# xarray-contrib/xeofs

Hardware: AMD Instinct MI355X
Metric: EOF randomized-SVD GB/s (algorithmic: 16 passes x n x p x 4 B per fit / fit time) (higher is better)
Workload: dtype f32 data, split-fp16 MFMA (f16x3+f16x3), f32 accumulate

## Files before the change

include/eofx.h:

```cpp
#ifndef EOFX_H
#define EOFX_H

#include <stdint.h>

#ifdef __cplusplus
extern "C" {
#endif

#define EOFX_ABI_VERSION 1
#define EOFX_MAX_SKETCH 256

#define EOFX_OK 0
#define EOFX_ERR_ARG (-1)
#define EOFX_ERR_HIP (-2)
#define EOFX_ERR_PARTIAL_NAN (-3)
#define EOFX_ERR_NAN_MISMATCH (-4)
#define EOFX_ERR_RANK (-5)
#define EOFX_ERR_LINALG (-6)
#define EOFX_ERR_NOMEM (-7)
#define EOFX_ERR_SHAPE (-8)

typedef struct eofx_ctx eofx_ctx;
typedef struct eofx_mat eofx_mat;

// ... 84 lines not shown
int eofx_ctx_last_iterations(const eofx_ctx *ctx, int *iterations);

int eofx_project_f32(eofx_ctx *ctx, const eofx_mat *m, const float *V, int k, float *out);
int eofx_reconstruct_f32(eofx_ctx *ctx, const float *S, const float *V, int64_t n, int64_t p,
                         int k, float *out);

int eofx_crosscov_rsvd_f32(eofx_ctx *ctx, const eofx_mat *x, const eofx_mat *y, int k,
                           int n_oversamples, int n_iter, const float *omega, int flip, float *Q1,
                           float *s, float *Q2, float *scores1, float *scores2, float *norm1,
                           float *norm2, double *tsc);
typedef const float *(*eofx_sketch_fn)(void *user);
int eofx_crosscov_rsvd_lazy_f32(eofx_ctx *ctx, const eofx_mat *x, const eofx_mat *y, int k, int n_oversamples,
                                int n_iter, eofx_sketch_fn omega_fn, void *omega_user, int flip, float *Q1, float *s,
                                float *Q2, float *scores1, float *scores2, float *norm1, float *norm2, double *tsc);

int eofx_panel_tmul_f32(eofx_ctx *ctx, const eofx_mat *m, const float *Zn, float *Yp, int L,
                        int precision);
int eofx_panel_mul_f32(eofx_ctx *ctx, const eofx_mat *m, const float *Yp, float *Wn, int L,
                       int precision);
int eofx_panel_gram_f64(eofx_ctx *ctx, const float *P, int64_t rows_pad, int L, double *G);
int eofx_panel_cholqr_f32(eofx_ctx *ctx, const float *P, int64_t rows_pad, int L, int l,
                          const double *G, float *out);
int eofx_panel_rinv_f64(eofx_ctx *ctx, const double *G, int L, int l, double *Rinv);
int eofx_panel_matmul_f32(eofx_ctx *ctx, const float *P, int64_t rows_pad, int L,
                          const double *M, int Lo, float *out);
int eofx_panel_colminmax_f32(eofx_ctx *ctx, const float *P, int64_t rows, int L, float *mx,
                             float *mn);
int eofx_panel_export_f32(eofx_ctx *ctx, const float *P, int64_t rows, int L, int k,
                          const double *sign, float *dst);
int eofx_panel_import_f32(eofx_ctx *ctx, const float *src, int64_t rows, int l, float *P,
                          int64_t rows_pad, int L);

int eofx_hilbert_f32(eofx_ctx *ctx, const eofx_mat *a, int padding, double decay_factor,
                     eofx_mat **out_imag, eofx_mat **out_real);
int eofx_mat_sumsq_f64(eofx_ctx *ctx, const eofx_mat *m, double *out);
int eofx_panel_rownorm_f64(eofx_ctx *ctx, const float *P, int64_t rows, int L, double *out);
int eofx_mat_feature_norms_f64(eofx_ctx *ctx, const eofx_mat *m, double *out);
int eofx_mat_sample_norms_f64(eofx_ctx *ctx, const eofx_mat *m, double *out);
int eofx_resample_f32(eofx_ctx *ctx, const eofx_mat *src, const int64_t *rows, int64_t n_rows, int center,
                      eofx_mat **out, double *mean, double *total_variance);
int eofx_panel_bootstrap_f32(eofx_ctx *ctx, const float *P_in, int64_t n, int64_t rows_pad, int L, const int64_t *idx,
                             const int64_t *order, const int64_t *rowptr, int transpose, float *P_out);
int eofx_lag_stats_f64(eofx_ctx *ctx, const eofx_mat *m, int tau, int embedding, double *mean, double *total_variance);
int eofx_lag_tmul_f32(eofx_ctx *ctx, const eofx_mat *m, int tau, int embedding, const double *mean, const float *Zn, int L,
                      float *Ye, int prec);
int eofx_lag_mul_f32(eofx_ctx *ctx, const eofx_mat *m, int tau, int embedding, const double *mean, const float *Ye, int L,
// ... 58 lines not shown
```

xeofs_amd/_lib.py:

```python

from __future__ import annotations

import ctypes as C
import os

import numpy as np

_HERE = os.path.dirname(os.path.abspath(__file__))
LIB_PATH = os.environ.get("EOFX_LIB") or os.path.join(_HERE, "lib", "libeofx.so")

EOFX_OK = 0
ERR_ARG, ERR_HIP, ERR_PARTIAL_NAN, ERR_NAN_MISMATCH, ERR_RANK, ERR_LINALG, ERR_NOMEM, ERR_SHAPE = (
    -1, -2, -3, -4, -5, -6, -7, -8)

_vp = C.c_void_p
_i64 = C.c_int64
_int = C.c_int
_pi64 = C.POINTER(C.c_int64)
_pd = C.POINTER(C.c_double)

SKETCH_FN = C.CFUNCTYPE(C.c_void_p, C.c_void_p)

ALLREDUCE_FN = C.CFUNCTYPE(C.c_int, C.c_void_p, C.c_void_p, C.c_int64, C.c_int, C.c_int, C.c_void_p)

# ... 8 lines not shown
    "eofx_ctx_set_precision": (_int, [_vp, _int, _int]),
    "eofx_ctx_profile": (_int, [_vp, _int]),
    "eofx_ctx_profile_read": (_int, [_vp, _pi64, _pd, _pd, _pd]),
    "eofx_ctx_profile_by_kernel": (_int, [_vp, _pi64, _pd]),
    "eofx_preprocess_f32": (_int, [_vp, _vp, _i64, _i64, _int, _int, _vp, _int, C.POINTER(_vp),
                                   _vp, _vp, _vp, _vp, _pi64, _pi64, _pd]),
    "eofx_apply_f32": (_int, [_vp, _vp, _i64, _i64, _vp, _vp, _vp, _vp, _int, C.POINTER(_vp), _vp, _pi64]),
    "eofx_mat_from_dense_f32": (_int, [_vp, _vp, _i64, _i64, _i64, C.POINTER(_vp)]),
    "eofx_mat_destroy": (_int, [_vp, _vp]),
    "eofx_mat_shape": (_int, [_vp, _pi64, _pi64, _pi64, _pi64]),
    "eofx_mat_download_f32": (_int, [_vp, _vp, _vp]),
    "eofx_rsvd_f32": (_int, [_vp, _vp, _int, _int, _int, _vp, _int, _vp, _vp, _vp]),
    "eofx_project_f32": (_int, [_vp, _vp, _vp, _int, _vp]),
    "eofx_reconstruct_f32": (_int, [_vp, _vp, _vp, _i64, _i64, _int, _vp]),
    "eofx_crosscov_rsvd_f32": (_int, [_vp, _vp, _vp, _int, _int, _int, _vp, _int, _vp, _vp, _vp, _vp,
                                      _vp, _vp, _vp, _pd]),
    "eofx_crosscov_rsvd_lazy_f32": (_int, [_vp, _vp, _vp, _int, _int, _int, SKETCH_FN, _vp, _int, _vp, _vp, _vp, _vp,
                                           _vp, _vp, _vp, _pd]),
    "eofx_panel_tmul_f32": (_int, [_vp, _vp, _vp, _vp, _int, _int]),
    "eofx_panel_mul_f32": (_int, [_vp, _vp, _vp, _vp, _int, _int]),
    "eofx_panel_gram_f64": (_int, [_vp, _vp, _i64, _int, _vp]),
    "eofx_panel_cholqr_f32": (_int, [_vp, _vp, _i64, _int, _int, _vp, _vp]),
    "eofx_panel_rinv_f64": (_int, [_vp, _vp, _int, _int, _vp]),
    "eofx_panel_matmul_f32": (_int, [_vp, _vp, _i64, _int, _vp, _int, _vp]),
    "eofx_panel_colminmax_f32": (_int, [_vp, _vp, _i64, _int, _vp, _vp]),
    "eofx_panel_export_f32": (_int, [_vp, _vp, _i64, _int, _int, _vp, _vp]),
    "eofx_panel_import_f32": (_int, [_vp, _vp, _i64, _int, _vp, _i64, _int]),
    "eofx_hilbert_f32": (_int, [_vp, _vp, _int, C.c_double, C.POINTER(_vp), C.POINTER(_vp)]),
    "eofx_mat_sumsq_f64": (_int, [_vp, _vp, _pd]),
    "eofx_fit_f32": (_int, [_vp, _vp, _i64, _i64, _int, _int, _vp, _int, _int, _int, _int, _vp, _i64, _int,
                            C.POINTER(_vp), _vp, _vp, _vp, _vp, _pi64, _pi64, _pd, _vp, _vp, _vp, C.POINTER(C.c_int)]),
    "eofx_fit_first_f32": (_int, [_vp, _vp, _i64, _i64, _int, _int, _vp, _int, _vp, _int, _int, _vp, C.POINTER(_vp),
                                  _vp, _vp, _vp, _vp, _pi64, _pi64, _pd, C.POINTER(C.c_int)]),
    "eofx_ctx_fit_info": (_int, [_vp, _pd]),
    "eofx_ctx_last_iterations": (_int, [_vp, C.POINTER(_int)]),
    "eofx_comm_unique_id": (_int, [C.c_char_p]),
    "eofx_ctx_comm_init_rccl": (_int, [_vp, C.c_char_p, _int, _int]),
    "eofx_ctx_comm_set_callback": (_int, [_vp, ALLREDUCE_FN, _vp, _int, _int]),
    "eofx_ctx_comm_clear": (_int, [_vp]),
    "eofx_ctx_comm_stats": (_int, [_vp, _pi64, _pi64, _pd]),
    "eofx_ctx_comm_selftest": (_int, [_vp, C.POINTER(C.c_int)]),
    "eofx_ctx_comm_probe": (_int, [_vp, _int, _vp, _vp, _int, _vp, _vp]),
    "eofx_fit_sharded_f32": (_int, [_vp, _vp, _i64, _i64, _i64, _int, _int, _vp, _int, _int, _int, _vp, _i64, _int,
                                    C.POINTER(_vp), _vp, _vp, _vp, _pd, _vp, _vp, _vp]),
    "eofx_ctx_comm_allreduce_f64": (_int, [_vp, _vp, _i64, _int]),
    "eofx_crosscov_rsvd_sharded_f32": (_int, [_vp, _vp, _vp, _i64, _i64, _i64, _i64, _int, _int, _int, _vp, _int, _vp, _vp,
# ... 103 lines not shown
```

xeofs_amd/csrc/eofx_abi.hip:

```cpp
#include <chrono>
#include "eofx_hfft.hpp"
#include "eofx_kernels.hpp"
#include "eofx_fit.hpp"
#include "eofx_gram.hpp"
#include "eofx_axb_dma.hpp"
#include "eofx_hosteig.hpp"
#include "eofx_lag.hpp"
#include "eofx_gw.hpp"
#include "eofx_spca.hpp"
#include "eofx_lagcov.hpp"
#ifndef EOFX_AXB_DMA_DEFAULT
#define EOFX_AXB_DMA_DEFAULT 1
#endif

#if !defined(__HIP_DEVICE_COMPILE__)
#include <immintrin.h>
#endif
#include <algorithm>
#include <array>
#include <atomic>
#include <cmath>
#include <complex>
#include <cstdarg>
#include <cstdio>
// ... 74 lines not shown
    int kind;
    ProfEvent(hipEvent_t a, hipEvent_t b, int k = 0) : first(a), second(b), kind(k) {}
  };
  std::vector<ProfEvent> prof_events;
  int64_t prof_kind_launches[3] = {0, 0, 0};
  double prof_kind_ms[3] = {0.0, 0.0, 0.0};
  double prof_flops = 0.0;
  double prof_bytes = 0.0;
  unsigned* amax_slots = nullptr;
  int amax_next = 0, amax_depth = 0;
  std::vector<std::pair<const float*, const unsigned*>> amax_known;
  double* pinned = nullptr;
  struct GramPlanDev {
    int nti = 0, ntj = 0, nst = 0;
    bool sym = false;
    GramPlan pl;
    GramItem* items = nullptr;
    int2* tiles = nullptr;
  };
  std::vector<GramPlanDev*> gram_plans;
  _Float16* axb_planes = nullptr;
  size_t axb_planes_bytes = 0;
  int axb_dma = -1;
  double fit_info[4] = {0.0, 0.0, 0.0, 0.0};
  int last_iters = 0;
  EofxComm* comm = nullptr;
};
constexpr int EOFX_AMAX_SLOTS = 1024;
constexpr int EOFX_HILBERT_OP_MAX_N = 16384;
constexpr size_t EOFX_PINNED_DOUBLES = 2 * 256 * 256 + 64;

struct eofx_mat {
  int64_t n = 0, p = 0, n_pad = 0, p_pad = 0;
  float* X = nullptr;
  float* Xt = nullptr;
  const float* raw = nullptr;
  float* raw_owned = nullptr;
  size_t raw_owned_bytes = 0;
  int64_t raw_ld = 0;
  float* aff = nullptr;
  unsigned* absmax_dev = nullptr;
  float absmax = 0.f;
  bool masked = false;
  int64_t p_valid = 0;
  int* act = nullptr;
  int64_t n_act = -1;
// ... 141 lines not shown
    std::lock_guard<std::mutex> g(g_fence[device].reg_mu);
    g_fence[device].ctxs.push_back(ctx);
  }
  *out = ctx;
  return EOFX_OK;
}
extern "C" int eofx_ctx_destroy(eofx_ctx* ctx) {
  if (!ctx) return EOFX_OK;
  {
    FenceGuard fence(ctx, false);
    if (ctx->device >= 0 && ctx->device < EOFX_MAX_DEVICES) {
      std::lock_guard<std::mutex> g(g_fence[ctx->device].reg_mu);
      auto& v = g_fence[ctx->device].ctxs;
      v.erase(std::remove(v.begin(), v.end(), ctx), v.end());
    }
  }
  (void)hipSetDevice(ctx->device);
  if (ctx->arena) {
    (void)hipStreamSynchronize(ctx->stream);
    (void)hipFree(ctx->arena);
  }
  pool_trim(ctx);
  if (ctx->amax_slots) (void)hipFree(ctx->amax_slots);
  if (ctx->pinned) (void)hipHostFree(ctx->pinned);
  for (auto& e : ctx->fft_plans) {
    hipfftDestroy((hipfftHandle)e.second.first);
    hipfftDestroy((hipfftHandle)e.second.second);
  }
  (void)eofx_ctx_comm_clear(ctx);
  if (ctx->axb_planes) (void)hipFree(ctx->axb_planes);
  for (auto* g : ctx->gram_plans) {
    if (g->items) (void)hipFree(g->items);
    if (g->tiles) (void)hipFree(g->tiles);
    delete g;
  }
  for (auto& h : ctx->hops) (void)eofx_mat_destroy(ctx, h.m);
  ctx->hops.clear();
  for (auto& h : ctx->hsetups) {
    if (h.chat) (void)hipFree(h.chat);
    if (h.hperm) (void)hipFree(h.hperm);
    if (h.u) (void)hipFree(h.u);
  }
  delete ctx;
  return EOFX_OK;
}
extern "C" int eofx_ctx_set_stream(eofx_ctx* ctx, void* stream) {
// ... 582 lines not shown
    if (masked)
      hipLaunchKernelGGL((axb_f16_kernel<4, 0, true>), dim3(gx, nfull), dim3(256), 0, ctx->stream, raw, ld, (int)rows, cols, aff, aff_ld, Y,
                         L, out, L, rows_pad, K, plan.kps, plan.S, rt, 0, a_scale, bmax, act);
    else
      hipLaunchKernelGGL(axb_f16_kernel<4>, dim3(gx, nfull), dim3(256), 0, ctx->stream, raw, ld, (int)rows, cols, aff, aff_ld, Y, L, out,
                         L, rows_pad, K, plan.kps, plan.S, rt, 0, a_scale, bmax);
    KCHK();
  }
  if (!dma && rem) {
    if (masked)
      hipLaunchKernelGGL((axb_f16_kernel<2, 0, true>), dim3(gx, 1), dim3(256), 0, ctx->stream, raw, ld, (int)rows, cols, aff, aff_ld, Y, L,
                         out, L, rows_pad, K, plan.kps, plan.S, rt, nfull * 64, a_scale, bmax, act);
    else
      hipLaunchKernelGGL(axb_f16_kernel<2>, dim3(gx, 1), dim3(256), 0, ctx->stream, raw, ld, (int)rows, cols, aff, aff_ld, Y, L, out,
                         L, rows_pad, K, plan.kps, plan.S, rt, nfull * 64, a_scale, bmax);
    KCHK();
  }
  if (ctx->profile) {
    HIPCHK(hipEventRecord(ev1, ctx->stream));
    ctx->prof_events.emplace_back(ev0, ev1, 1);
    ctx->prof_flops += 2.0 * (double)K * (double)rows_pad * (double)L;
    ctx->prof_bytes += (double)K * (double)rows * 4.0 * (nfull + (rem ? 1 : 0));
  }
  if (plan.S > 1) {
    const int64_t count4 = rows_pad * L / 4;
    hipLaunchKernelGGL(splitk_reduce_kernel, dim3((int)std::min<int64_t>((count4 + 255) / 256, amax_out ? 2048 : 4096)), dim3(256), 0,
                       ctx->stream, out, W, count4, plan.S, amax_out);
    KCHK();
  }
  return EOFX_OK;
}

static int gram_parts(int64_t rows, int L) {
  const int64_t by_rows = std::min<int64_t>((rows + 127) / 128, 256);
  const int64_t by_mem = ((int64_t)128 << 20) / ((int64_t)L * L * 8);
  if (const char* ev = std::getenv("EOFX_GRAM_PARTS")) return std::max(1, atoi(ev));
  return (int)std::max<int64_t>(1, std::min(by_rows, std::max<int64_t>(by_mem, 1)));
}

static int launch_gram(eofx_ctx* ctx, const float* P, int64_t rows, int L, double* G) {
  const int nb = (L + 63) / 64;
  const int nbx = gram_parts(rows, L);
  ArenaScope scope(ctx);
  ARENA(double, part, (size_t)nbx * L * L);
  hipLaunchKernelGGL(gram_mfma_kernel, dim3(nbx, nb * nb), dim3(256), 0, ctx->stream, P, rows, L, part);
  KCHK();
  const int64_t count = (int64_t)L * L;
// ... 73 lines not shown
    if (dead[c]) continue;
    X[(size_t)c * l + c] = 1.0 / A[(size_t)c * l + c];
    for (int r = c - 1; r >= 0; --r) {
      double sum = 0.0;
      for (int t = r + 1; t <= c; ++t) sum += A[(size_t)r * l + t] * X[(size_t)t * l + c];
      X[(size_t)r * l + c] = -sum / A[(size_t)r * l + r];
    }
  }
  for (int r = 0; r < L; ++r)
    for (int c = 0; c < L; ++c) Rinv[(size_t)r * L + c] = (r < l && c < l) ? X[(size_t)r * l + c] : 0.0;
}

static int launch_rinv(eofx_ctx* ctx, const double* G, int L, int l, double* Rinv);
static size_t rinv_blocked_bytes(int l);
static bool matmul_nt_ok(int64_t rows, int L, int Lo);
static size_t matmul_nt_scratch(eofx_ctx* ctx, int64_t rows, int L, int Lo);
static int launch_matmul_nt(eofx_ctx* ctx, const float* P, int64_t rows, int L, const double* Mx, int Lo, float* out);
static int launch_cholqr(eofx_ctx* ctx, const float* P, int64_t rows, int L, int l, const double* G,
                         float* out) {
  ArenaScope scope(ctx);
  ARENA(double, Rinv, (size_t)L * L);
  CHK(launch_rinv(ctx, G, L, l, Rinv));
  return launch_matmul(ctx, P, rows, L, Rinv, L, out, true);
}

static int launch_colminmax(eofx_ctx* ctx, const float* P, int64_t rows, int L, float* mx, float* mn) {
  const int nparts = (int)std::max<int64_t>(1, std::min<int64_t>((rows + 127) / 128, 1024));
  ArenaScope scope(ctx);
  ARENA(float, pmx, (size_t)nparts * L);
  ARENA(float, pmn, (size_t)nparts * L);
  hipLaunchKernelGGL(colminmax_part_kernel, dim3(nparts, (L + 63) / 64), dim3(256), 0, ctx->stream, P,
                     rows, L, pmx, pmn);
  KCHK();
  hipLaunchKernelGGL(colminmax_final_kernel, dim3((L + 63) / 64), dim3(256), 0, ctx->stream, pmx, pmn,
                     nparts, L, mx, mn);
  KCHK();
  return EOFX_OK;
}

static int export_panel(eofx_ctx* ctx, const float* P, int64_t rows, int L, int k, const double* sign,
                        float* dst) {
  if (!dst) return EOFX_OK;
  ArenaScope scope(ctx);
  double* dsign = nullptr;
  if (sign) {
    dsign = arena_alloc<double>(ctx, k);
// ... 808 lines not shown
  ENTER(ctx);
  CHK(arena_reserve(ctx, atb_scratch_bytes(m->n_pad, round_up(m->p, ATB_KG), L)));
  return panel_mul(ctx, m, Yp, Wn, L, prec);
}
extern "C" int eofx_panel_gram_f64(eofx_ctx* ctx, const float* P, int64_t rows_pad, int L, double* G) {
  if (!ctx || !P || !G || L % 32) return set_err(ctx, EOFX_ERR_ARG, "bad argument");
  ENTER(ctx);
  CHK(arena_reserve(ctx, (size_t)(4 * gram_parts(rows_pad, L) + 1) * L * L * sizeof(double)));
  return launch_gram(ctx, P, rows_pad, L, G);
}
extern "C" int eofx_panel_cholqr_f32(eofx_ctx* ctx, const float* P, int64_t rows_pad, int L, int l,
                                     const double* G, float* out) {
  if (!ctx || !P || !G || !out || P == out) return set_err(ctx, EOFX_ERR_ARG, "bad argument");
  ENTER(ctx);
  CHK(arena_reserve(ctx, (size_t)2 * L * L * sizeof(double) + (l > 64 ? rinv_blocked_bytes(l) : 0)));
  return launch_cholqr(ctx, P, rows_pad, L, l, G, out);
}
extern "C" int eofx_panel_rinv_f64(eofx_ctx* ctx, const double* G, int L, int l, double* Rinv) {
  if (!ctx || !G || !Rinv || L <= 0 || l <= 0 || l > L || G == Rinv) return set_err(ctx, EOFX_ERR_ARG, "bad argument");
  ENTER(ctx);
  if (l > 64) CHK(arena_reserve(ctx, rinv_blocked_bytes(l)));
  return launch_rinv(ctx, G, L, l, Rinv);
}
extern "C" int eofx_panel_matmul_f32(eofx_ctx* ctx, const float* P, int64_t rows_pad, int L,
                                     const double* M, int Lo, float* out) {
  if (!ctx || !P || !M || !out || P == out) return set_err(ctx, EOFX_ERR_ARG, "bad argument");
  ENTER(ctx);
  if (matmul_nt_ok(rows_pad, L, Lo)) {
    const size_t need = matmul_nt_scratch(ctx, rows_pad, L, Lo);
    if (need && arena_reserve(ctx, need) == EOFX_OK) return launch_matmul_nt(ctx, P, rows_pad, L, M, Lo, out);
  }
  return launch_matmul(ctx, P, rows_pad, L, M, Lo, out);
}
extern "C" int eofx_panel_colminmax_f32(eofx_ctx* ctx, const float* P, int64_t rows, int L, float* mx,
                                        float* mn) {
  if (!ctx || !P || !mx || !mn) return set_err(ctx, EOFX_ERR_ARG, "bad argument");
  if (L <= 0 || L % 4 || rows < 0)
    return set_err(ctx, EOFX_ERR_ARG, "colminmax: L=%d must be a positive multiple of 4, rows=%lld non-negative", L, (long long)rows);
  ENTER(ctx);
  CHK(arena_reserve(ctx, (size_t)2 * 1024 * L * sizeof(float) + 4096));
  return launch_colminmax(ctx, P, rows, L, mx, mn);
}
extern "C" int eofx_panel_export_f32(eofx_ctx* ctx, const float* P, int64_t rows, int L, int k,
                                     const double* sign, float* dst) {
  if (!ctx || !P || !dst || k > L) return set_err(ctx, EOFX_ERR_ARG, "bad argument");
  ENTER(ctx);
  CHK(arena_reserve(ctx, (size_t)rows * k * sizeof(float) + 8192));
  return export_panel(ctx, P, rows, L, k, sign, dst);
}
extern "C" int eofx_panel_import_f32(eofx_ctx* ctx, const float* src, int64_t rows, int l, float* P,
                                     int64_t rows_pad, int L) {
  if (!ctx || !P || !src || l > L || rows > rows_pad) return set_err(ctx, EOFX_ERR_ARG, "bad argument");
  if (L <= 0 || L % 4 || l < 0 || rows < 0)
    return set_err(ctx, EOFX_ERR_ARG, "import: L=%d must be a positive multiple of 4, l=%d and rows=%lld non-negative", L, l, (long long)rows);
  ENTER(ctx);
  CHK(arena_reserve(ctx, (size_t)rows * l * sizeof(float) + 8192));
  return import_panel(ctx, src, rows, l, P, rows_pad, L);
}

struct LinOp {
  int64_t tall, small, tall_pad, small_pad;
  std::function<int(const float*, float*, int, int)> fwd;
  std::function<int(const float*, float*, int, int)> bwd;
  std::function<int(double*, int64_t)> reduce_tall_gram;
  std::function<int(double*, int64_t)> reduce_small_gram;
  int64_t rule_tall_pad = 0;
};

struct RsvdOut {
  float* Tvec;
  float* Svec;
  int Lo;
  std::vector<double> s;
  int64_t tall_pad = 0, small_pad = 0;
};

static int rsvd_auto_iters(int k, int64_t n, int64_t p) {
  return ((double)k < 0.1 * (double)std::min(n, p)) ? 7 : 4;
}

constexpr size_t EOFX_ORTH_TALL_BYTES = (size_t)16 << 20;
constexpr double EOFX_PEAKED_RATIO = 30.0;
static bool orth_tall_rule(int64_t tall_pad, int L, int prec_power) {
  if (std::getenv("EOFX_FORCE_ORTH_TALL")) return true;
  return prec_power == EOFX_PREC_F64 || (size_t)tall_pad * L * sizeof(float) <= EOFX_ORTH_TALL_BYTES;
}
extern "C" int eofx_orth_tall_rule(int64_t tall_rows_pad, int L, int prec_power) {
  return orth_tall_rule(tall_rows_pad, L, prec_power) ? 1 : 0;
}
// ... 125 lines not shown
  bool first_done = false;
  auto fwd = [&](const float* z, float* y, int prec) -> int {
    if (first_fwd && !first_done) {
      first_done = true;
      return (*first_fwd)(z, y, L);
    }
    first_done = true;
    return op.fwd(z, y, L, prec);
  };
  auto gram_tall = [&](const float* Pn, double* Gout) -> int {
    CHK(launch_gram(ctx, Pn, op.tall_pad, L, Gout));
    return op.reduce_tall_gram ? op.reduce_tall_gram(Gout, (int64_t)L * L) : EOFX_OK;
  };
  auto gram_small = [&](const float* Pn, double* Gout) -> int {
    CHK(launch_gram(ctx, Pn, op.small_pad, L, Gout));
    return op.reduce_small_gram ? op.reduce_small_gram(Gout, (int64_t)L * L) : EOFX_OK;
  };
  const int pp = ctx->prec_power, pf = ctx->prec_final;
  const bool orth_always = orth_tall_rule(op.rule_tall_pad > 0 ? op.rule_tall_pad : op.tall_pad, L, pp);
  bool orth_rest = orth_always;
  hipEvent_t peaked_ev = nullptr;
  bool peaked_pending = false;
  int rc = EOFX_OK;
  for (int it = 0; it < (range ? 0 : n_iter) && rc == EOFX_OK; ++it) {
    rc = fwd(Zs, Yt, pp);
    if (rc != EOFX_OK) break;
    if (peaked_pending) {
      peaked_pending = false;
      if (hipEventSynchronize(peaked_ev) != hipSuccess) rc = set_err(ctx, EOFX_ERR_HIP, "event wait failed");
      else orth_rest = eofx_peaked_spectrum(pin, L, l) != 0;
      if (rc != EOFX_OK) break;
    }
    if (it == 0 || orth_rest) {
      if ((rc = gram_tall(Yt, G)) != EOFX_OK) break;
      if ((rc = launch_cholqr(ctx, Yt, op.tall_pad, L, l, G, Qt)) != EOFX_OK) break;
      rc = op.bwd(Qt, Ws, L, pp);
    } else {
      rc = op.bwd(Yt, Ws, L, pp);
    }
    if (rc != EOFX_OK) break;
    const bool ask = it == 0 && !orth_always && n_iter > 1;
    if ((rc = gram_small(Ws, ask ? G0 : G)) != EOFX_OK) break;
    if (ask) {
      if (hipMemcpyAsync(pin, G0, sizeof(double) * L * L, hipMemcpyDeviceToHost, ctx->stream) != hipSuccess ||
          (!peaked_ev && hipEventCreateWithFlags(&peaked_ev, hipEventDisableTiming) != hipSuccess) ||
          hipEventRecord(peaked_ev, ctx->stream) != hipSuccess) {
        rc = set_err(ctx, EOFX_ERR_HIP, "asynchronous Gram download failed");
        break;
      }
      peaked_pending = true;
    }
    rc = launch_cholqr(ctx, Ws, op.small_pad, L, l, ask ? G0 : G, Zs);
  }
  if (peaked_ev) {
    if (peaked_pending) (void)hipEventSynchronize(peaked_ev);
    (void)hipEventDestroy(peaked_ev);
  }
  if (rc != EOFX_OK) return rc;
  if (range) CHK((*range)(Zs, Yt, L));
  else CHK(fwd(Zs, Yt, pp));
  CHK(gram_tall(Yt, G));
  CHK(launch_cholqr(ctx, Yt, op.tall_pad, L, l, G, Qt));
  CHK(gram_tall(Qt, G));
  CHK(launch_rinv(ctx, G, L, l, R2));
  CHK(op.bwd(Qt, Zs, L, pf));
  CHK(launch_matmul(ctx, Zs, op.small_pad, L, R2, L, Ws));
  CHK(gram_small(Ws, G));
  double* hG = pin;
  double* hR2 = pin + (size_t)L * L;
  HIPCHK(hipMemcpyAsync(hG, G, sizeof(double) * L * L, hipMemcpyDeviceToHost, ctx->stream));
  HIPCHK(hipMemcpyAsync(hR2, R2, sizeof(double) * L * L, hipMemcpyDeviceToHost, ctx->stream));
  HIPCHK(hipStreamSynchronize(ctx->stream));
  std::vector<double> Gl((size_t)l * l), w(l), Uh((size_t)l * l);
  for (int i = 0; i < l; ++i)
    for (int j = 0; j < l; ++j) {
// ... 212 lines not shown
                             const float* omega, int flip, float* U, float* s, float* V) {
  if (!ctx || !m || !omega || k <= 0 || n_oversamples < 0) return set_err(ctx, EOFX_ERR_ARG, "bad argument");
  ENTER(ctx);
  const int64_t n = m->n, p = m->p, r = std::min(n, p);
  if (k > r)
    return set_err(ctx, EOFX_ERR_RANK,
                   "n_modes must be less than or equal to the rank of the dataset (rank = %lld).", (long long)r);
  const int l_req = k + n_oversamples;
  const int l = (int)std::min<int64_t>(l_req, r);
  if (l > EOFX_MAX_SKETCH)
    return set_err(ctx, EOFX_ERR_ARG, "sketch width k+n_oversamples = %d > %d is not supported", l, EOFX_MAX_SKETCH);
  if (n_iter < 0) n_iter = rsvd_auto_iters(k, n, p);
  const bool transposed = n < p;
  LinOp op;
  if (transposed) {
    op = {p, n, m->p_pad, m->n_pad,
          [&](const float* z, float* y, int L, int pr) { return panel_tmul(ctx, m, z, y, L, pr); },
          [&](const float* y, float* w, int L, int pr) { return panel_mul(ctx, m, y, w, L, pr); }};
  } else {
    op = {n, p, m->n_pad, m->p_pad,
          [&](const float* z, float* y, int L, int pr) { return panel_mul(ctx, m, z, y, L, pr); },
          [&](const float* y, float* w, int L, int pr) { return panel_tmul(ctx, m, y, w, L, pr); }};
  }
  CHK(arena_reserve(ctx, rsvd_scratch_bytes(op.tall_pad, op.small_pad, l, k)));
  ArenaScope scope(ctx);
  std::vector<float> om_clamped;
  const float* om = omega;
  if (l == r) {
    om_clamped.assign((size_t)op.small * l, 0.f);
    for (int64_t i = 0; i < l; ++i) om_clamped[(size_t)i * l + i] = 1.f;
    om = om_clamped.data();
  } else if (l != l_req) {
    if (is_device_ptr(omega)) return set_err(ctx, EOFX_ERR_ARG, "omega must be a host pointer");
    om_clamped.resize((size_t)op.small * l);
    for (int64_t i = 0; i < op.small; ++i)
      for (int j = 0; j < l; ++j) om_clamped[(size_t)i * l + j] = omega[(size_t)i * l_req + j];
    om = om_clamped.data();
  }
  RsvdOut ro;
  CHK(rsvd_core(ctx, op, k, l, n_iter, om, ro));
  return rsvd_finish(ctx, ro, transposed, n, p, k, flip, U, s, V);
}

struct FitFirst {
  eofx_ctx* ctx = nullptr;
  const float* Xd = nullptr;
// ... 208 lines not shown
  }
};

static bool fit_first_eligible(const eofx_ctx* ctx, const float* Xdev, int64_t n, int64_t P, int l) {
  return ctx->keep_raw == 2 && ctx->prec_power == EOFX_PREC_F16X3 && n < P && l > 0 && l < n && round_up(l, 32) <= 64 &&
         l % 32 != 0 && P % 4 == 0 && ((uintptr_t)Xdev % 16) == 0 && n < ((int64_t)1 << 31) && !std::getenv("EOFX_NO_FUSED_FIT");
}

static int fit_fused(eofx_ctx* ctx, const float* Xd, int64_t n, int64_t P, int center, int standardize,
                     const double* feat_weights, int k, int l, int n_iter, const float* omega, int flip,
                     eofx_mat** out, double* mean, double* std_, double* total_variance, float* U, float* s, float* V,
                     uint8_t* valid_feature, int64_t* p_valid) {
  const int64_t p_pad = round_up(P, ATB_BM), n_pad = round_up(n, ATB_BM);
  CHK(arena_reserve(ctx, rsvd_scratch_bytes(p_pad, n_pad, l, k) + FitFirst::bytes(n, P, l)));
  ArenaScope scope(ctx);
  FitFirst ff;
  int rc = ff.prepare(ctx, Xd, n, P, center, standardize, feat_weights, l);
  if (rc != EOFX_OK) return rc;
  FirstFwd first = [&](const float* Zs, float* Yt, int LL) -> int { return ff.run(Zs, Yt, LL); };
  const eofx_mat* m = ff.m;
  LinOp op = {P, n, p_pad, n_pad,
              [&](const float* z, float* y, int LL, int pr) { return panel_tmul(ctx, m, z, y, LL, pr); },
              [&](const float* y, float* w, int LL, int pr) { return panel_mul(ctx, m, y, w, LL, pr); }};
  RsvdOut ro;
  rc = rsvd_core(ctx, op, k, l, n_iter, omega, ro, &first);
  if (rc != EOFX_OK) return rc;
  CHK(rsvd_finish(ctx, ro, true, n, P, k, flip, U, s, V));
  CHK(ff.valid_features(valid_feature));
  if (p_valid) *p_valid = ff.m->masked ? ff.m->p_valid : P;
  return ff.finish(mean, std_, total_variance, out);
}

extern "C" int eofx_fit_first_f32(eofx_ctx* ctx, const float* X, int64_t n, int64_t P, int center, int standardize,
                                  const double* feat_weights, int check_nans, const float* Zn, int L, int l, float* Yp,
                                  eofx_mat** out, double* mean, double* std_, uint8_t* valid_feature, uint8_t* valid_sample,
                                  int64_t* n_out, int64_t* p_out, double* total_variance, int* fused) {
  if (!ctx || !X || !out || !Zn || !Yp || n <= 0 || P <= 0 || L <= 0 || L % 32 || l <= 0 || l > L)
    return set_err(ctx, EOFX_ERR_ARG, "bad argument");
  ENTER(ctx);
  if (fused) *fused = 0;
  ctx->fit_info[0] = ctx->fit_info[1] = ctx->fit_info[2] = 0.0;
  Staged st;
  CHK(stage_input(ctx, X, (size_t)n * P, st));
  if (fit_first_eligible(ctx, st.dev, n, P, l) && round_up(l, 32) == L) {
    CHK(arena_reserve(ctx, FitFirst::bytes(n, P, l) + atb_scratch_bytes(round_up(P, ATB_BM), round_up(n, ATB_KG), L)));
    ArenaScope scope(ctx);
// ... 3519 lines not shown
```

xeofs_amd/csrc/eofx_kernels.hpp:

```cpp
#pragma once
#include <hip/hip_runtime.h>
#include <stdint.h>

namespace eofx {

typedef float f32x16 __attribute__((ext_vector_type(16)));
typedef float f32x4 __attribute__((ext_vector_type(4)));
typedef float f32x2 __attribute__((ext_vector_type(2)));

__device__ __forceinline__ void aff_split(double sh, float& hi, float& lo) {
  hi = (float)sh;
  lo = (float)(sh - (double)hi);
}
__device__ __forceinline__ float aff_map(float x, float sh_hi, float sh_lo, float scale) {
  return ((x - sh_hi) - sh_lo) * scale;
}
__device__ __forceinline__ float aff_fma(float x, float sh_hi, float s, float nls) {
  return __builtin_fmaf(x - sh_hi, s, nls);
}

__device__ __forceinline__ void amax_commit(float mx, unsigned* __restrict__ amax_out) {
  __shared__ float amax_red_[16];
#pragma unroll
  for (int o = 32; o > 0; o >>= 1) mx = fmaxf(mx, __shfl_xor(mx, o));
// ... 1174 lines not shown

__global__ __launch_bounds__(256) void cproj_embed_kernel(const double* __restrict__ C, int nb, int LP, double* __restrict__ E) {
  const int h = LP / 2;
  const int64_t total = (int64_t)nb * h * h;
  for (int64_t t = (int64_t)blockIdx.x * blockDim.x + threadIdx.x; t < total; t += (int64_t)gridDim.x * blockDim.x) {
    const int b = (int)(t / (h * h)), i = (int)(t / h % h), j = (int)(t % h);
    const double* Cb = C + (int64_t)b * LP * LP;
    double* Eb = E + (int64_t)b * LP * LP;
    const double rr = Cb[i * LP + j], ii = Cb[(h + i) * LP + h + j], ri = Cb[i * LP + h + j], ir = Cb[(h + i) * LP + j];
    const double cr = rr + ii, ci = ri - ir;
    Eb[i * LP + j] = cr;
    Eb[(h + i) * LP + j] = -ci;
    Eb[i * LP + h + j] = ci;
    Eb[(h + i) * LP + h + j] = cr;
  }
}

__device__ __forceinline__ double rl_f64(double v, int lane) {
  const int lo = __builtin_amdgcn_readlane(__double2loint(v), lane);
  const int hi = __builtin_amdgcn_readlane(__double2hiint(v), lane);
  return __hiloint2double(hi, lo);
}

__global__ __launch_bounds__(256) void chol_rinv_kernel(const double* __restrict__ G, int L, int l,
                                                         double* __restrict__ Rinv, double tol,
                                                         const double* __restrict__ d0_ext = nullptr,
                                                         unsigned long long* __restrict__ prof = nullptr) {
#define EOFX_RINV_T(i) do { if (prof && threadIdx.x == 0) prof[i] = wall_clock64(); } while (0)
  EOFX_RINV_T(0);
  __shared__ double A[64][65];
  __shared__ double X[64][65];
  __shared__ double d0s[64], pivs[64];
  __shared__ double Tm[3][16][17];
  __shared__ int dead[64];
  const int tid = threadIdx.x;
  for (int i = tid; i < 64 * 64; i += 256) {
    const int r = i >> 6, c = i & 63;
    double v = (r == c) ? 1.0 : 0.0;
    if (r <= c && c < l) v = G[(int64_t)r * L + c];
    A[r][c] = v;
  }
  if (tid < 64) {
    d0s[tid] = (tid < l) ? (d0_ext ? d0_ext[tid] : G[(int64_t)tid * L + tid]) : 1.0;
    pivs[tid] = 1.0;
    dead[tid] = 0;
  }
  __syncthreads();
  EOFX_RINV_T(1);
  for (int jb = 0; jb < l; jb += 8) {
    const int je = jb + 8;
// ... 71 lines not shown
#pragma unroll 16
          for (int m = 0; m < 16; ++m) t += A[16 * i + rr][16 * k + m] * X[16 * k + m][16 * j + cc];
        Tm[i][rr][cc] = t;
      }
      __syncthreads();
      for (int i = 0; i + d < 4; ++i) {
        const int j = i + d;
        double x = 0.0;
#pragma unroll 16
        for (int m = 0; m < 16; ++m) x += X[16 * i + rr][16 * i + m] * Tm[i][m][cc];
        X[16 * i + rr][16 * j + cc] = -x;
      }
      __syncthreads();
    }
  }
  __syncthreads();
  EOFX_RINV_T(3);
  for (int i = tid; i < 64 * 64; i += 256) {
    const int r = i >> 6, c = i & 63;
    if (r < L && c < L) Rinv[(int64_t)r * L + c] = (r <= c && c < l && !dead[c]) ? X[r][c] : 0.0;
  }
  EOFX_RINV_T(4);
#undef EOFX_RINV_T
}

template <bool TA>
__global__ __launch_bounds__(256) void dgemm64_kernel(const double* __restrict__ A, int lda, const double* B, int ldb,
                                                       double* C, int ldc, int K, double alpha, double beta, int upper,
                                                       int64_t sA = 0, int64_t sB = 0, int64_t sC = 0) {
  __shared__ double As[16][65], Bs[16][65];
  const int bx = blockIdx.x, by = blockIdx.y;
  if (upper && by > bx) return;
  A += (int64_t)blockIdx.z * sA;
  B += (int64_t)blockIdx.z * sB;
  C += (int64_t)blockIdx.z * sC;
  const int tx = threadIdx.x & 15, ty = threadIdx.x >> 4;
  double acc[4][4];
#pragma unroll
  for (int i = 0; i < 4; ++i)
#pragma unroll
    for (int j = 0; j < 4; ++j) acc[i][j] = 0.0;
  for (int k0 = 0; k0 < K; k0 += 16) {
#pragma unroll
    for (int e = 0; e < 4; ++e) {
      const int idx = threadIdx.x + 256 * e;
      if (TA) {
// ... 1340 lines not shown
```

xeofs_amd/engine.py:

```python

from __future__ import annotations

import contextlib
import ctypes as C
import numbers

import numpy as np

from . import _lib
from ._lib import ptr, raise_for


def _f32c(a):
    if isinstance(a, np.ndarray):
        return np.ascontiguousarray(a, dtype=np.float32)
    if hasattr(a, "data_ptr"):
        import torch

        if a.dtype != torch.float32 or not a.is_contiguous():
            a = a.to(torch.float32).contiguous()
        return a
    return np.ascontiguousarray(np.asarray(a), dtype=np.float32)


# ... 725 lines not shown
    L = Yp.shape[1]
    if out is None:
        out = torch.empty((mat.n_pad, L), dtype=torch.float32, device=Yp.device)
    raise_for(ctx.lib.eofx_panel_mul_f32(ctx.handle, mat.handle, ptr(Yp), ptr(out), L, _lib.PREC[prec]), ctx.handle)
    return out


def panel_gram(ctx: Context, P, out=None):
    torch = _torch()
    L = P.shape[1]
    if out is None:
        out = torch.empty((L, L), dtype=torch.float64, device=P.device)
    raise_for(ctx.lib.eofx_panel_gram_f64(ctx.handle, ptr(P), P.shape[0], L, ptr(out)), ctx.handle)
    return out


def panel_cholqr(ctx: Context, P, l: int, G, out=None):
    torch = _torch()
    if out is None:
        out = torch.empty_like(P)
    raise_for(ctx.lib.eofx_panel_cholqr_f32(ctx.handle, ptr(P), P.shape[0], P.shape[1], int(l), ptr(G), ptr(out)),
              ctx.handle)
    return out


def panel_rinv(ctx: Context, G, l: int):
    torch = _torch()
    out = torch.empty_like(G)
    raise_for(ctx.lib.eofx_panel_rinv_f64(ctx.handle, ptr(G), G.shape[0], int(l), ptr(out)), ctx.handle)
    return out


def panel_matmul(ctx: Context, P, M, out=None):
    torch = _torch()
    Lo = M.shape[1]
    if out is None:
        out = torch.empty((P.shape[0], Lo), dtype=torch.float32, device=P.device)
    raise_for(ctx.lib.eofx_panel_matmul_f32(ctx.handle, ptr(P), P.shape[0], P.shape[1], ptr(M), Lo, ptr(out)),
              ctx.handle)
    return out


def panel_colminmax(ctx: Context, P, rows: int):
    torch = _torch()
    L = P.shape[1]
    mx = torch.empty(L, dtype=torch.float32, device=P.device)
# ... 341 lines not shown
```

Baseline: 5905.

## Fuse split-K reduce, small Gram, and Cholesky inverse into one kernel

In the randomized-SVD power iteration, the backward product's split-K reduction is deferred and fused with the small-side Gram computation (f64 MFMA), a last-block ticket reduction of per-block Gram partials, and the Cholesky/R-inverse into a single kernel launch. The old path ran a separate reduce kernel, a Gram kernel, and a cholqr path. This removes several kernel launches and one full read of the reduced panel. In exchange it adds a global atomic ticket with release/acquire fences and last-block serial work, and exposes a test entry point plus an environment switch to turn it off.

```diff
diff --git a/include/eofx.h b/include/eofx.h
--- a/include/eofx.h
+++ b/include/eofx.h
@@ -130,6 +130,8 @@
 int eofx_panel_cholqr_f32(eofx_ctx *ctx, const float *P, int64_t rows_pad, int L, int l,
                           const double *G, float *out);
 int eofx_panel_rinv_f64(eofx_ctx *ctx, const double *G, int L, int l, double *Rinv);
+int eofx_panel_small_step_f32(eofx_ctx *ctx, const float *part, int splits, int64_t rows_pad, int l, int fused,
+                              float *Ws, double *G, double *Rinv, float *Zs, unsigned *amax);
 int eofx_panel_matmul_f32(eofx_ctx *ctx, const float *P, int64_t rows_pad, int L,
                           const double *M, int Lo, float *out);
 int eofx_panel_colminmax_f32(eofx_ctx *ctx, const float *P, int64_t rows, int L, float *mx,
diff --git a/xeofs_amd/_lib.py b/xeofs_amd/_lib.py
--- a/xeofs_amd/_lib.py
+++ b/xeofs_amd/_lib.py
@@ -54,6 +54,7 @@
     "eofx_panel_gram_f64": (_int, [_vp, _vp, _i64, _int, _vp]),
     "eofx_panel_cholqr_f32": (_int, [_vp, _vp, _i64, _int, _int, _vp, _vp]),
     "eofx_panel_rinv_f64": (_int, [_vp, _vp, _int, _int, _vp]),
+    "eofx_panel_small_step_f32": (_int, [_vp, _vp, _int, _i64, _int, _int, _vp, _vp, _vp, _vp, _vp]),
     "eofx_panel_matmul_f32": (_int, [_vp, _vp, _i64, _int, _vp, _int, _vp]),
     "eofx_panel_colminmax_f32": (_int, [_vp, _vp, _i64, _int, _vp, _vp]),
     "eofx_panel_export_f32": (_int, [_vp, _vp, _i64, _int, _int, _vp, _vp]),
diff --git a/xeofs_amd/csrc/eofx_abi.hip b/xeofs_amd/csrc/eofx_abi.hip
--- a/xeofs_amd/csrc/eofx_abi.hip
+++ b/xeofs_amd/csrc/eofx_abi.hip
@@ -120,6 +120,13 @@
   _Float16* axb_planes = nullptr;
   size_t axb_planes_bytes = 0;
   int axb_dma = -1;
+  struct AxbDefer {
+    const float* W = nullptr;
+    const float* part = nullptr;
+    int S = 0;
+  };
+  AxbDefer* axb_defer = nullptr;
+  unsigned* step_ticket = nullptr;
   double fit_info[4] = {0.0, 0.0, 0.0, 0.0};
   int last_iters = 0;
   EofxComm* comm = nullptr;
@@ -307,6 +314,7 @@
   }
   pool_trim(ctx);
   if (ctx->amax_slots) (void)hipFree(ctx->amax_slots);
+  if (ctx->step_ticket) (void)hipFree(ctx->step_ticket);
   if (ctx->pinned) (void)hipHostFree(ctx->pinned);
   for (auto& e : ctx->fft_plans) {
     hipfftDestroy((hipfftHandle)e.second.first);
@@ -935,7 +943,10 @@
     ctx->prof_flops += 2.0 * (double)K * (double)rows_pad * (double)L;
     ctx->prof_bytes += (double)K * (double)rows * 4.0 * (nfull + (rem ? 1 : 0));
   }
-  if (plan.S > 1) {
+  if (plan.S > 1 && ctx->axb_defer && ctx->axb_defer->W == W) {
+    ctx->axb_defer->part = out;
+    ctx->axb_defer->S = plan.S;
+  } else if (plan.S > 1) {
     const int64_t count4 = rows_pad * L / 4;
     hipLaunchKernelGGL(splitk_reduce_kernel, dim3((int)std::min<int64_t>((count4 + 255) / 256, amax_out ? 2048 : 4096)), dim3(256), 0,
                        ctx->stream, out, W, count4, plan.S, amax_out);
@@ -1055,6 +1066,24 @@
   ARENA(double, Rinv, (size_t)L * L);
   CHK(launch_rinv(ctx, G, L, l, Rinv));
   return launch_matmul(ctx, P, rows, L, Rinv, L, out, true);
+}
+
+static int launch_small_step(eofx_ctx* ctx, const float* part, int splits, float* Ws, int64_t rows, int l, double* gpart, double* G,
+                             double* Rinv, unsigned* amax_ws) {
+  if (rows <= 0 || rows >= ((int64_t)1 << 40) || l <= 0 || l > 64 || splits < 1) return set_err(ctx, EOFX_ERR_ARG, "small step: bad geometry");
+  if (!ctx->step_ticket) {
+    HIPCHK(hipMalloc((void**)&ctx->step_ticket, 256));
+    HIPCHK(hipMemsetAsync(ctx->step_ticket, 0, 256, ctx->stream));
+  }
+  const int nbx = gram_parts(rows, 64);
+  hipLaunchKernelGGL(small_step_kernel, dim3(nbx), dim3(256), 0, ctx->stream, part, splits, Ws, part != Ws ? 1 : 0, rows, l, gpart, G, Rinv,
+                     1e-13, ctx->step_ticket, amax_ws);
+  KCHK();
+  return EOFX_OK;
+}
+static bool small_step_off() {
+  const char* ev = std::getenv("EOFX_SMALL_STEP");
+  return ev && atoi(ev) == 0;
 }
 
 static int launch_colminmax(eofx_ctx* ctx, const float* P, int64_t rows, int L, float* mx, float* mn) {
@@ -1909,6 +1938,28 @@
   if (l > 64) CHK(arena_reserve(ctx, rinv_blocked_bytes(l)));
   return launch_rinv(ctx, G, L, l, Rinv);
 }
+extern "C" int eofx_panel_small_step_f32(eofx_ctx* ctx, const float* part, int splits, int64_t rows_pad, int l, int fused, float* Ws,
+                                         double* G, double* Rinv, float* Zs, unsigned* amax) {
+  if (!ctx || !part || !Ws || !G || !Rinv || !Zs || part == Ws || Ws == Zs || splits < 1 || rows_pad <= 0 || l <= 0 ||
+      l > 64)
+    return set_err(ctx, EOFX_ERR_ARG, "bad argument");
+  ENTER(ctx);
+  const int L = 64;
+  CHK(arena_reserve(ctx, (size_t)(4 * gram_parts(rows_pad, L) + 2) * L * L * sizeof(double)));
+  ArenaScope scope(ctx);
+  if (fused) {
+    ARENA(double, gpart, (size_t)gram_parts(rows_pad, L) * L * L);
+    CHK(launch_small_step(ctx, part, splits, Ws, rows_pad, l, gpart, G, Rinv, amax));
+  } else {
+    const int64_t count4 = rows_pad * L / 4;
+    hipLaunchKernelGGL(splitk_reduce_kernel, dim3((int)std::min<int64_t>((count4 + 255) / 256, 2048)), dim3(256), 0, ctx->stream, part, Ws,
+                       count4, splits, amax);
+    KCHK();
+    CHK(launch_gram(ctx, Ws, rows_pad, L, G));
+    CHK(launch_rinv(ctx, G, L, l, Rinv));
+  }
+  return launch_matmul(ctx, Ws, rows_pad, L, Rinv, L, Zs, true);
+}
 extern "C" int eofx_panel_matmul_f32(eofx_ctx* ctx, const float* P, int64_t rows_pad, int L,
                                      const double* M, int Lo, float* out) {
   if (!ctx || !P || !M || !out || P == out) return set_err(ctx, EOFX_ERR_ARG, "bad argument");
@@ -1952,6 +2003,7 @@
   std::function<int(double*, int64_t)> reduce_tall_gram;
   std::function<int(double*, int64_t)> reduce_small_gram;
   int64_t rule_tall_pad = 0;
+  bool bwd_is_product = false;
 };
 
 struct RsvdOut {
@@ -2123,6 +2175,13 @@
   hipEvent_t peaked_ev = nullptr;
   bool peaked_pending = false;
   int rc = EOFX_OK;
+  const bool fuse_small = op.bwd_is_product && L == 64 && l <= 64 && !op.reduce_small_gram && !op.reduce_tall_gram && !range &&
+                          !small_step_off();
+  double *step_part = nullptr, *step_rinv = nullptr;
+  if (fuse_small) {
+    step_part = arena_alloc<double>(ctx, (size_t)gram_parts(op.small_pad, L) * L * L);
+    step_rinv = arena_alloc<double>(ctx, (size_t)L * L);
+  }
   for (int it = 0; it < (range ? 0 : n_iter) && rc == EOFX_OK; ++it) {
     rc = fwd(Zs, Yt, pp);
     if (rc != EOFX_OK) break;
@@ -2132,16 +2191,28 @@
       else orth_rest = eofx_peaked_spectrum(pin, L, l) != 0;
       if (rc != EOFX_OK) break;
     }
+    const bool ask = it == 0 && !orth_always && n_iter > 1;
+    const bool fused = step_part && step_rinv;
+    eofx_ctx::AxbDefer defer;
+    defer.W = Ws;
+    if (fused) ctx->axb_defer = &defer;
     if (it == 0 || orth_rest) {
-      if ((rc = gram_tall(Yt, G)) != EOFX_OK) break;
-      if ((rc = launch_cholqr(ctx, Yt, op.tall_pad, L, l, G, Qt)) != EOFX_OK) break;
-      rc = op.bwd(Qt, Ws, L, pp);
+      if ((rc = gram_tall(Yt, G)) == EOFX_OK && (rc = launch_cholqr(ctx, Yt, op.tall_pad, L, l, G, Qt)) == EOFX_OK)
+        rc = op.bwd(Qt, Ws, L, pp);
     } else {
       rc = op.bwd(Yt, Ws, L, pp);
     }
+    ctx->axb_defer = nullptr;
     if (rc != EOFX_OK) break;
-    const bool ask = it == 0 && !orth_always && n_iter > 1;
-    if ((rc = gram_small(Ws, ask ? G0 : G)) != EOFX_OK) break;
+    if (fused) {
+      const bool split = defer.S > 1;
+      const float* amax_ws = split ? amax_get(ctx, Ws) : nullptr;
+      rc = launch_small_step(ctx, split ? defer.part : Ws, split ? defer.S : 1, Ws, op.small_pad, l, step_part, ask ? G0 : G, step_rinv,
+                             reinterpret_cast<unsigned*>(const_cast<float*>(amax_ws)));
+      if (rc != EOFX_OK) break;
+    } else if ((rc = gram_small(Ws, ask ? G0 : G)) != EOFX_OK) {
+      break;
+    }
     if (ask) {
       if (hipMemcpyAsync(pin, G0, sizeof(double) * L * L, hipMemcpyDeviceToHost, ctx->stream) != hipSuccess ||
           (!peaked_ev && hipEventCreateWithFlags(&peaked_ev, hipEventDisableTiming) != hipSuccess) ||
@@ -2151,7 +2222,8 @@
       }
       peaked_pending = true;
     }
-    rc = launch_cholqr(ctx, Ws, op.small_pad, L, l, ask ? G0 : G, Zs);
+    if (fused) rc = launch_matmul(ctx, Ws, op.small_pad, L, step_rinv, L, Zs, true);
+    else rc = launch_cholqr(ctx, Ws, op.small_pad, L, l, ask ? G0 : G, Zs);
   }
   if (peaked_ev) {
     if (peaked_pending) (void)hipEventSynchronize(peaked_ev);
@@ -2410,6 +2482,7 @@
           [&](const float* z, float* y, int L, int pr) { return panel_mul(ctx, m, z, y, L, pr); },
           [&](const float* y, float* w, int L, int pr) { return panel_tmul(ctx, m, y, w, L, pr); }};
   }
+  op.bwd_is_product = true;
   CHK(arena_reserve(ctx, rsvd_scratch_bytes(op.tall_pad, op.small_pad, l, k)));
   ArenaScope scope(ctx);
   std::vector<float> om_clamped;
@@ -2664,6 +2737,7 @@
   LinOp op = {P, n, p_pad, n_pad,
               [&](const float* z, float* y, int LL, int pr) { return panel_tmul(ctx, m, z, y, LL, pr); },
               [&](const float* y, float* w, int LL, int pr) { return panel_mul(ctx, m, y, w, LL, pr); }};
+  op.bwd_is_product = true;
   RsvdOut ro;
   rc = rsvd_core(ctx, op, k, l, n_iter, omega, ro, &first);
   if (rc != EOFX_OK) return rc;
diff --git a/xeofs_amd/csrc/eofx_kernels.hpp b/xeofs_amd/csrc/eofx_kernels.hpp
--- a/xeofs_amd/csrc/eofx_kernels.hpp
+++ b/xeofs_amd/csrc/eofx_kernels.hpp
@@ -1220,10 +1220,10 @@
   return __hiloint2double(hi, lo);
 }
 
-__global__ __launch_bounds__(256) void chol_rinv_kernel(const double* __restrict__ G, int L, int l,
-                                                         double* __restrict__ Rinv, double tol,
-                                                         const double* __restrict__ d0_ext = nullptr,
-                                                         unsigned long long* __restrict__ prof = nullptr) {
+__device__ __forceinline__ void chol_rinv_body(const double* __restrict__ G, int L, int l,
+                                               double* __restrict__ Rinv, double tol,
+                                               const double* __restrict__ d0_ext,
+                                               unsigned long long* __restrict__ prof) {
 #define EOFX_RINV_T(i) do { if (prof && threadIdx.x == 0) prof[i] = wall_clock64(); } while (0)
   EOFX_RINV_T(0);
   __shared__ double A[64][65];
@@ -1341,6 +1341,185 @@
   }
   EOFX_RINV_T(4);
 #undef EOFX_RINV_T
+}
+__global__ __launch_bounds__(256) void chol_rinv_kernel(const double* __restrict__ G, int L, int l,
+                                                         double* __restrict__ Rinv, double tol,
+                                                         const double* __restrict__ d0_ext = nullptr,
+                                                         unsigned long long* __restrict__ prof = nullptr) {
+  chol_rinv_body(G, L, l, Rinv, tol, d0_ext, prof);
+}
+
+constexpr int SSTEP_CH = 8;
+__global__ __launch_bounds__(256) void small_step_kernel(const float* __restrict__ part, int splits, float* Ws, int write_ws,
+                                                          int64_t rows, int l, double* __restrict__ Gpart, double* G,
+                                                          double* __restrict__ Rinv, double tol, unsigned* __restrict__ ticket,
+                                                          unsigned* __restrict__ amax_out) {
+  const int tid = threadIdx.x;
+  const int lane = tid & 63, wave = tid >> 6;
+  const int lc = lane & 15, lk = lane >> 4;
+  const int64_t count4 = rows * 16;
+  const int64_t wstride = (int64_t)gridDim.x * 16;
+  const int64_t base = ((int64_t)blockIdx.x * 4 + wave) * 4;
+  const int64_t nsub = base < rows ? 4 * ((rows - base + 4 * wstride - 1) / (4 * wstride)) : 0;
+  f64x4 acc[4][4];
+#pragma unroll
+  for (int x = 0; x < 4; ++x)
+#pragma unroll
+    for (int y = 0; y < 4; ++y) acc[x][y] = f64x4{0.0, 0.0, 0.0, 0.0};
+  float mx = 0.f;
+  const f32x4* part4 = reinterpret_cast<const f32x4*>(part);
+  for (int64_t d0 = 0; d0 < nsub; d0 += SSTEP_CH) {
+    int64_t idx[SSTEP_CH];
+    bool live[SSTEP_CH];
+#pragma unroll
+    for (int u = 0; u < SSTEP_CH; ++u) {
+      const int64_t r = base + lk + (d0 + u) * wstride;
+      live[u] = r < rows;
+      idx[u] = (live[u] ? r : rows - 1) * 16 + lc;
+    }
+    double a[SSTEP_CH][4];
+#pragma unroll
+    for (int u = 0; u < SSTEP_CH; ++u)
+#pragma unroll
+      for (int e = 0; e < 4; ++e) a[u][e] = 0.0;
+#pragma unroll 4
+    for (int s = 0; s < splits; ++s) {
+      f32x4 v[SSTEP_CH];
+#pragma unroll
+      for (int u = 0; u < SSTEP_CH; ++u) v[u] = part4[(int64_t)s * count4 + idx[u]];
+#pragma unroll
+      for (int u = 0; u < SSTEP_CH; ++u)
+#pragma unroll
+        for (int e = 0; e < 4; ++e) a[u][e] += v[u][e];
+    }
+#pragma unroll
+    for (int u = 0; u < SSTEP_CH; ++u) {
+      f32x4 o = {(float)a[u][0], (float)a[u][1], (float)a[u][2], (float)a[u][3]};
+      if (live[u]) {
+        if (write_ws) {
+          reinterpret_cast<f32x4*>(Ws)[idx[u]] = o;
+          mx = fmaxf(mx, fmaxf(fmaxf(fabsf(o[0]), fabsf(o[1])), fmaxf(fabsf(o[2]), fabsf(o[3]))));
+        }
+      } else {
+        o = f32x4{0.f, 0.f, 0.f, 0.f};
+      }
+      if (d0 + u < nsub) {
+#pragma unroll
+        for (int x = 0; x < 4; ++x)
+#pragma unroll
+          for (int y = x; y < 4; ++y)
+            acc[x][y] = __builtin_amdgcn_mfma_f64_16x16x4f64((double)o[x], (double)o[y], acc[x][y], 0, 0, 0);
+      }
+    }
+  }
+  if (write_ws && amax_out) amax_commit(mx, amax_out);
+  __shared__ double Gs[64][65];
+  __shared__ int last_;
+  for (int w = 0; w < 4; ++w) {
+    if (wave == w) {
+#pragma unroll
+      for (int x = 0; x < 4; ++x)
+#pragma unroll
+        for (int y = x; y < 4; ++y) {
+#pragma unroll
+          for (int q = 0; q < 4; ++q) {
+            const int i = 4 * (lk + 4 * q) + x, j = 4 * lc + y;
+            if (w == 0) {
+              Gs[i][j] = acc[x][y][q];
+              if (x < y) Gs[j][i] = acc[x][y][q];
+            } else {
+              Gs[i][j] += acc[x][y][q];
+              if (x < y) Gs[j][i] += acc[x][y][q];
+            }
+          }
+        }
+    }
+    __syncthreads();
+  }
+  double* Gp = Gpart + (int64_t)blockIdx.x * 4096;
+  for (int e = tid; e < 4096; e += 256) {
+    const int i = e >> 6, j = e & 63;
+    if (i <= (j | 1)) Gp[e] = Gs[i][j];
+  }
+  asm volatile("s_waitcnt vmcnt(0)" ::: "memory");
+  __syncthreads();
+  if (tid == 0) {
+    __builtin_amdgcn_fence(__ATOMIC_RELEASE, "agent");
+    asm volatile("s_waitcnt vmcnt(0)" ::: "memory");
+    const unsigned t = __hip_atomic_fetch_add(ticket, 1u, __ATOMIC_RELAXED, __HIP_MEMORY_SCOPE_AGENT);
+    const int last = t == gridDim.x - 1;
+    if (last) {
+      __builtin_amdgcn_fence(__ATOMIC_ACQUIRE, "agent");
+      asm volatile("s_waitcnt vmcnt(0)" ::: "memory");
+    }
+    last_ = last;
+  }
+  __syncthreads();
+  if (!last_) return;
+  {
+    const int nparts = (int)gridDim.x;
+    constexpr int NI = 5;
+    int off[NI];
+    bool ok[NI];
+#pragma unroll
+    for (int m = 0; m < NI; ++m) {
+      const int k = tid + 256 * m;
+      ok[m] = k < 32 * 33;
+      const int kk = ok[m] ? k : 0;
+      const int sr = kk / 33, t = kk % 33, n0 = 32 - sr / 2;
+      const int i = t < n0 ? sr : 63 - sr;
+      const int jp = t < n0 ? sr / 2 + t : (63 - sr) / 2 + (t - n0);
+      off[m] = 64 * i + 2 * jp;
+    }
+    double s[NI][4][2];
+#pragma unroll
+    for (int m = 0; m < NI; ++m)
+#pragma unroll
+      for (int q = 0; q < 4; ++q) s[m][q][0] = s[m][q][1] = 0.0;
+    typedef double f64x2 __attribute__((ext_vector_type(2)));
+    int b = 0;
+#pragma unroll 2
+    for (; b + 4 <= nparts; b += 4) {
+      f64x2 v[NI][4];
+#pragma unroll
+      for (int m = 0; m < NI; ++m)
+#pragma unroll
+        for (int q = 0; q < 4; ++q) v[m][q] = *reinterpret_cast<const f64x2*>(Gpart + (int64_t)(b + q) * 4096 + off[m]);
+#pragma unroll
+      for (int m = 0; m < NI; ++m)
+#pragma unroll
+        for (int q = 0; q < 4; ++q) {
+          s[m][q][0] += v[m][q][0];
+          s[m][q][1] += v[m][q][1];
+        }
+    }
+#pragma unroll
+    for (int q = 0; q < 3; ++q) {
+      if (b + q >= nparts) break;
+#pragma unroll
+      for (int m = 0; m < NI; ++m) {
+        const f64x2 v = *reinterpret_cast<const f64x2*>(Gpart + (int64_t)(b + q) * 4096 + off[m]);
+        s[m][q][0] += v[0];
+        s[m][q][1] += v[1];
+      }
+    }
+#pragma unroll
+    for (int m = 0; m < NI; ++m) {
+      if (!ok[m]) continue;
+      const int i = off[m] >> 6, j = off[m] & 63;
+#pragma unroll
+      for (int h = 0; h < 2; ++h) {
+        const double g = ((s[m][0][h] + s[m][1][h]) + s[m][2][h]) + s[m][3][h];
+        if (i <= j + h) {
+          G[64 * i + j + h] = g;
+          if (i < j + h) G[64 * (j + h) + i] = g;
+        }
+      }
+    }
+    if (tid == 0) __hip_atomic_store(ticket, 0u, __ATOMIC_RELAXED, __HIP_MEMORY_SCOPE_AGENT);
+  }
+  __syncthreads();
+  chol_rinv_body(G, 64, l, Rinv, tol, nullptr, nullptr);
 }
 
 template <bool TA>
diff --git a/xeofs_amd/engine.py b/xeofs_amd/engine.py
--- a/xeofs_amd/engine.py
+++ b/xeofs_amd/engine.py
@@ -771,6 +771,19 @@
     raise_for(ctx.lib.eofx_panel_cholqr_f32(ctx.handle, ptr(P), P.shape[0], P.shape[1], int(l), ptr(G), ptr(out)),
               ctx.handle)
     return out
+
+
+def panel_small_step(ctx: Context, part, l: int, fused: bool):
+    torch = _torch()
+    splits, rows, L = part.shape
+    Ws = torch.empty((rows, L), dtype=torch.float32, device=part.device)
+    Zs = torch.empty_like(Ws)
+    G = torch.empty((L, L), dtype=torch.float64, device=part.device)
+    Rinv = torch.empty_like(G)
+    amax = torch.zeros(1, dtype=torch.int32, device=part.device)
+    raise_for(ctx.lib.eofx_panel_small_step_f32(ctx.handle, ptr(part), int(splits), rows, int(l), int(bool(fused)), ptr(Ws),
+                                                ptr(G), ptr(Rinv), ptr(Zs), ptr(amax)), ctx.handle)
+    return Ws, G, Rinv, Zs, amax
 
 
 def panel_rinv(ctx: Context, G, l: int):
```

Measured after the change: 5866. No clear change (-0.7%).
